# audioku/meta-transfer-learning

Hardware: AMD Instinct MI355X
Metric: meta-steps/sec (higher is better)
Workload: dtype f32 (emulated: 3x3 conv + input Linear on 2 x fp16 pieces "h2" = 22 significand bits, big GEMMs and attention (d_k = 64) on 3 x bf16 pieces "x3" = exact fp32 operands, small products on fp32 MFMA, element-wise on VALU; fp32 accumulation everywhere)

## Files before the change

meta-transfer-learning_amd/csrc/mtl_mfma.hip:

```cpp
#include <cstdlib>
#include <type_traits>

#include "mtl_common.h"
#include "mtl_h2.h"
#include "mtl_conv_narrow.h"
#include "../../include/mtl_hip.h"

namespace {

constexpr int BK = 32;
constexpr int NT = 256;

template <int ROWS>
struct LdsK {
    static constexpr int LD = BK + 1;
    static constexpr int SIZE = ROWS * LD;
    static __device__ __forceinline__ int at(int row, int k) { return row * LD + k; }
};
template <int ROWS>
struct LdsMN {
    static constexpr int LD = ROWS + 4;
    static constexpr int SIZE = BK * LD;
    static __device__ __forceinline__ int at(int row, int k) { return k * LD + row; }
};
// ... 782 lines not shown
    mx = wave_max(mx);
    if ((threadIdx.x & 63) == 0) sh[threadIdx.x >> 6] = mx;
    __syncthreads();
    if (threadIdx.x == 0) hdr_f[1 + blockIdx.x] = fmaxf(fmaxf(sh[0], sh[1]), fmaxf(sh[2], sh[3]));
}

struct ConvX3P {
    const float* x;
    const uint8_t* am_in;
    const unsigned char* w3;
    const float* bias;
    const float* act;
    float* y;
    uint8_t* am_out;
    ConvGeom g;
    int ntile;
    int dbg;
    int ntf, ntt, tiles;
    const float* amax_in;
    float* amax_out;
    int Bt;
    long sW, sBias, sAmaxIn, sAmaxOut;
    const int* widths;
    int wshift;
#ifdef MTL_X3_PROF
    unsigned long long* prof;
#endif
};
#ifdef MTL_X3_PROF
static unsigned long long* g_x3_prof = nullptr;
extern "C" void mtl_x3_prof_set(void* buf) { g_x3_prof = (unsigned long long*)buf; }
#define X3_T(v) const unsigned long long v = __builtin_amdgcn_s_memtime()
#define X3_ACC(slot, a, b) prof_acc[slot] += (b) - (a)
#define X3_PROF_DECL unsigned long long prof_acc[8] = {0, 0, 0, 0, 0, 0, 0, 0}
#define X3_PROF_FLUSH()                                                                                    \
    if (p.prof && (threadIdx.x & 63) == 0) {                                                               \
        for (int k_ = 0; k_ < 8; ++k_) p.prof[((long)blockIdx.x * 16 + (threadIdx.x >> 6)) * 8 + k_] = prof_acc[k_]; \
    }
#else
#define X3_T(v)
#define X3_ACC(slot, a, b)
#define X3_PROF_DECL
#define X3_PROF_FLUSH()
#endif

constexpr int XH_HF = 18;

struct X3Tile {
    int b, n0, t0, f0;
};

inline int device_cu_count() {
    int dev = 0, n = 0;
    if (hipGetDevice(&dev) != hipSuccess || hipDeviceGetAttribute(&n, hipDeviceAttributeMultiprocessorCount, dev) != hipSuccess || n <= 0)
        n = 256;
    return n;
}

template <int G>
__device__ inline int x3_task_rows(const ConvX3P& p, int task) {
    const int r = ((p.widths[task] >> p.wshift) + 8 * G - 1) / (8 * G);
    return r < p.ntt ? (r < 1 ? 1 : r) : p.ntt;
}

template <int G>
__device__ inline int x3_total_tiles(const ConvX3P& p) {
    if (!p.widths) return p.tiles;
    const int nt = p.g.B / p.Bt;
    int total = 0;
    for (int k = 0; k < nt; ++k) total += p.Bt * p.ntile * x3_task_rows<G>(p, k) * p.ntf;
    return total;
}

struct X3Cur {
    int k = 0, lo = 0, hi = -1, ntt = 0;
};

template <int G>
__device__ inline X3Tile x3_tile(const ConvX3P& p, int id, X3Cur& c) {
    X3Tile t;
    int ntt = p.ntt, b0 = 0;
    if (p.widths) {
        const int per_row = p.Bt * p.ntile * p.ntf, nt = p.g.B / p.Bt;
        if (c.hi < 0 || id < c.lo) {
            c.k = 0;
            c.lo = 0;
            c.ntt = x3_task_rows<G>(p, 0);
            c.hi = per_row * c.ntt;
        }
        while (id >= c.hi && c.k < nt - 1) {
            ++c.k;
            c.lo = c.hi;
            c.ntt = x3_task_rows<G>(p, c.k);
            c.hi = c.lo + per_row * c.ntt;
        }
        id -= c.lo;
        ntt = c.ntt;
        b0 = c.k * p.Bt;
    }
    const int fx = id % p.ntf;
    id /= p.ntf;
    const int ty = id % ntt;
    id /= ntt;
    t.f0 = fx * 16;
    t.t0 = ty * (8 * G);
    t.n0 = id % p.ntile;
    t.b = b0 + id / p.ntile;
    return t;
}

template <bool SWZ>
__device__ __forceinline__ float x3_wave_max(float v) {
    if constexpr (!SWZ) {
        return wave_max(v);
    } else {
        v = fmaxf(v, __int_as_float(__builtin_amdgcn_ds_swizzle(__float_as_int(v), (1 << 10) | 0x1f)));
        v = fmaxf(v, __int_as_float(__builtin_amdgcn_ds_swizzle(__float_as_int(v), (2 << 10) | 0x1f)));
        v = fmaxf(v, __int_as_float(__builtin_amdgcn_ds_swizzle(__float_as_int(v), (4 << 10) | 0x1f)));
        v = fmaxf(v, __int_as_float(__builtin_amdgcn_ds_swizzle(__float_as_int(v), (8 << 10) | 0x1f)));
        v = fmaxf(v, __int_as_float(__builtin_amdgcn_ds_swizzle(__float_as_int(v), (16 << 10) | 0x1f)));
        return fmaxf(__int_as_float(__builtin_amdgcn_readlane(__float_as_int(v), 0)), __int_as_float(__builtin_amdgcn_readlane(__float_as_int(v), 32)));
    }
}
template <bool SWZ>
__device__ __forceinline__ float x3_amax_read(const float* a) {
    return x3_wave_max<SWZ>(a[(threadIdx.x & (MTL_AMAX_SLOTS - 1)) * MTL_AMAX_STRIDE]);
}
template <bool SWZ>
__device__ __forceinline__ void x3_amax_raise(float* a, float mx) {
    mx = x3_wave_max<SWZ>(mx);
    float* slot = a + (blockIdx.x & (MTL_AMAX_SLOTS - 1)) * MTL_AMAX_STRIDE;
    if ((threadIdx.x & 63) == 0 && mx > *slot) atomicMax(reinterpret_cast<unsigned*>(slot), __float_as_uint(mx));
}

template <int BN, int G, bool UNPOOL, int EPI, int NP, int WN>
constexpr bool x3h_slim_fwd() {
    return X3H_M16 != 0 && NP == 2 && G == 2 && !UNPOOL &&
           ((BN == 64 && WN == 1 && EPI != EPI_DGRAD) || (BN == 128 && WN == 2 && EPI == EPI_RELU));
}
template <int BN, int G, bool UNPOOL, int EPI, int NP, int WN>
constexpr bool x3h_slim_dg128() {
    return NP == 2 && G == 2 && UNPOOL && EPI == EPI_DGRAD && BN == 128 && WN == 2;
}
constexpr bool x3h_lane_offsets_fit(long ch) { return (15 * ch + 64) * 4 < (1L << 32); }
static_assert(x3h_lane_offsets_fit(128) && x3h_lane_offsets_fit(71582783) && !x3h_lane_offsets_fit(71582784), "just below / at the limit");
static_assert((15 * 71582783L + 63) * 4 + 7 <= 0xffffffffL, "the last byte a lane offset reaches below the limit");

template <int BN, int G, bool UNPOOL, int EPI, int NP, int WN, bool WIDE = false>
__global__ __launch_bounds__((2 * WN * G + 4) * 64) __attribute__((amdgpu_waves_per_eu(WN == 1 ? 4 : 1)))
void conv3x3_x3h_kernel(ConvX3P p) {
    constexpr bool SLIM_FWD = !WIDE && x3h_slim_fwd<BN, G, UNPOOL, EPI, NP, WN>();
    constexpr bool SLIM_H32 = WN == 1 && EPI == EPI_DGRAD;
    constexpr bool SLIM_DG = SLIM_H32 || (!WIDE && x3h_slim_dg128<BN, G, UNPOOL, EPI, NP, WN>());
    constexpr bool SLIM_HALO = SLIM_DG;
    constexpr bool SLIM = SLIM_DG || SLIM_FWD;
    constexpr int CW = 2 * WN;
    constexpr int WTM = 64, WTN = BN / WN, TM = WTM / 32, TN = WTN / 32;
    constexpr int XH_HT = 8 * G + 2, XH_NPIX = XH_HT * XH_HF;
    constexpr int XH_APLANE = XH_NPIX * X3_ROWB;
    constexpr int NHALO = 3 * 64;
    constexpr int XH_NVA = (XH_NPIX * 8 + NHALO - 1) / NHALO;
    constexpr int NCONS = CW * G * 64;
    constexpr int BPLANE = BN * 64, BBUF = NP * BPLANE, ABUF = NP * XH_APLANE;
    constexpr int NDMA = BBUF / 1024;
    extern __shared__ __attribute__((aligned(16))) unsigned char smx[];
    unsigned char* smA = smx;
    unsigned char* smB = smx + ABUF;
    const int tid = threadIdx.x;
    const int Cin = p.g.Cin, Cout = p.g.Cout, cch = Cin / BK, nk = 9 * cch;
    const int T = p.g.T, F = p.g.F, Tp = p.g.Tp, Fp = p.g.Fp;
    const int my_tiles = (x3_total_tiles<G>(p) - (int)blockIdx.x + (int)gridDim.x - 1) / (int)gridDim.x;
    if (my_tiles <= 0) return;
    const int nstage = my_tiles * cch;
    const int nstep = nstage * 9;

    if (tid >= NCONS + 64) {
        const int ptid = tid - NCONS - 64;
        float sx = NP == 2 ? pow2_scale(x3_amax_read<SLIM>(p.amax_in)) : 1.f;
        int sx_task = 0;
        X3Cur cur_scale, cur_halo;
        auto set_scale = [&](int qc) {
            if (NP != 2 || p.Bt >= p.g.B) return;
            const int tk = x3_tile<G>(p, blockIdx.x + (qc / cch) * gridDim.x, cur_scale).b / p.Bt;
            if (tk != sx_task) {
                sx_task = tk;
                sx = pow2_scale(x3_amax_read<SLIM>(p.amax_in + tk * p.sAmaxIn));
            }
        };
        float4 hv[XH_NVA];
        uchar4 ha[XH_NVA];
        unsigned hm[SLIM_HALO ? 1 : XH_NVA];
        auto fetch_halo = [&](int q) {
            const int j = q / cch, c = q - j * cch;
            const X3Tile tl = x3_tile<G>(p, blockIdx.x + j * gridDim.x, cur_halo);
            int pt = ptid;
            if constexpr (SLIM_HALO) asm volatile("" : "+v"(pt));
#pragma unroll
            for (int i = 0; i < XH_NVA; ++i) {
                const int e = pt + i * NHALO;
                const int hp = min(e >> 3, XH_NPIX - 1), c4 = (e & 7) * 4;
                const int ht = hp / XH_HF, hf = hp - ht * XH_HF;
                const int ts = tl.t0 + ht - 1, fs = tl.f0 + hf - 1;
                bool ok = (e >> 3) < XH_NPIX && (unsigned)ts < (unsigned)T && (unsigned)fs < (unsigned)F;
                const int tc = min(max(ts, 0), T - 1), fc = min(max(fs, 0), F - 1);
                if (!UNPOOL) {
                    hv[i] = *reinterpret_cast<const float4*>(p.x + (((long)tl.b * T + tc) * F + fc) * Cin + c * BK + c4);
                    if constexpr (SLIM_HALO) hm[0] = i ? hm[0] | ((ok ? 1u : 0u) << i) : (ok ? 1u : 0u);
                    else hm[i] = ok ? 1u : 0u;
                } else {
                    const int tp = tc >> 1, fp = fc >> 1;
                    ok = ok && tp < Tp && fp < Fp;
                    if constexpr (SLIM_H32) {
                        const long sbase = (long)__builtin_amdgcn_readfirstlane(tl.b) * Tp * Fp * Cin + c * BK;
                        const unsigned o = (unsigned)((min(tp, Tp - 1) * Fp + min(fp, Fp - 1)) * Cin + c4);
                        ha[i] = *reinterpret_cast<const uchar4*>(p.am_in + sbase + o);
                        hv[i] = *reinterpret_cast<const float4*>(reinterpret_cast<const char*>(p.x + sbase) + o * 4u);
                    } else {
                    const long o = (((long)tl.b * Tp + min(tp, Tp - 1)) * Fp + min(fp, Fp - 1)) * Cin + c * BK + c4;
                    ha[i] = *reinterpret_cast<const uchar4*>(p.am_in + o);
                    hv[i] = *reinterpret_cast<const float4*>(p.x + o);
                    }
                    if constexpr (SLIM_HALO) hm[0] = i ? hm[0] | ((ok ? 1u : 0u) << i) : (ok ? 1u : 0u);
                    else hm[i] = (ok ? 1u : 0u) | ((unsigned)(((fs & 1) << 1) | (ts & 1)) << 1);
                }
            }
        };
        auto commit_halo = [&]() {
            int pt = ptid;
            if constexpr (SLIM_HALO) asm volatile("" : "+v"(pt));
#pragma unroll
            for (int i = 0; i < XH_NVA; ++i) {
                const int e = pt + i * NHALO;
                if ((e >> 3) >= XH_NPIX) continue;
                float4 v = hv[i];
                const bool ok = SLIM_HALO ? (hm[0] >> i) & 1u : hm[i] & 1u;
                if (!UNPOOL) {
                    v = mask4(v, ok ? 15u : 0u);
                } else {
                    const int ht_ = (e >> 3) / XH_HF, hf_ = (e >> 3) - ht_ * XH_HF;
                    const unsigned sub = SLIM_HALO ? (unsigned)((((hf_ + 1) & 1) << 1) | ((ht_ + 1) & 1)) : hm[SLIM_HALO ? 0 : i] >> 1;
                    v.x = (ok && ha[i].x == sub) ? v.x : 0.f;
                    v.y = (ok && ha[i].y == sub) ? v.y : 0.f;
                    v.z = (ok && ha[i].z == sub) ? v.z : 0.f;
                    v.w = (ok && ha[i].w == sub) ? v.w : 0.f;
                }
                uint2 pc[NP];
                split_x4<NP>(v, sx, pc);
                unsigned char* dst = smA + (e >> 3) * X3_ROWB + (e & 7) * 8;
#pragma unroll
                for (int q = 0; q < NP; ++q) *reinterpret_cast<uint2*>(dst + q * XH_APLANE) = pc[q];
            }
        };
        const bool doA = !(p.dbg & 2);
        X3_PROF_DECL;
        X3_T(h0);
        if (doA) fetch_halo(0);
        set_scale(0);
        if (doA) commit_halo();
        if (nstage > 1 && doA) fetch_halo(1);
        __syncthreads();
        X3_T(h1);
        X3_ACC(0, h0, h1);
#pragma unroll 1
        for (int q = 0; q < nstage; ++q) {
            X3_T(a0);
#pragma unroll 1
            for (int tap = 0; tap < 9; ++tap) __syncthreads();
            X3_T(a1);
            X3_ACC(1, a0, a1);
            if (q + 1 < nstage) {
                set_scale(q + 1);
                if (doA) commit_halo();
                X3_T(a2);
                X3_ACC(2, a1, a2);
                if (q + 2 < nstage && doA) fetch_halo(q + 2);
                X3_T(a3);
                X3_ACC(3, a2, a3);
                __syncthreads();
                X3_T(a4);
                X3_ACC(4, a3, a4);
            }
        }
        X3_PROF_FLUSH();
        return;
    }
    if (tid >= NCONS) {
        const int lane = tid & 63;
        const bool doB = !(p.dbg & 4);
        int dma_j = -1, dma_n0 = 0;
        X3Cur cur_dma;
        const unsigned char* dma_w3 = p.w3;
        auto dma = [&](int s_) {
            const int q = s_ / 9, tap = s_ - q * 9;
            const int j = q / cch, c = q - j * cch;
            if (j != dma_j && (p.ntile != 1 || p.Bt < p.g.B)) {
                const X3Tile tl = x3_tile<G>(p, blockIdx.x + j * gridDim.x, cur_dma);
                dma_n0 = tl.n0 * BN;
                dma_w3 = p.w3 + (tl.b / p.Bt) * p.sW;
                dma_j = j;
            }
            const int n0 = dma_n0;
            const unsigned char* w3 = dma_w3;
            const int kt = tap * cch + c;
            unsigned char* dst = smB + (s_ % 3) * BBUF;
#pragma unroll
            for (int i = 0; i < NDMA; ++i) {
                const int piece = i / (BN / 16), r16 = i - piece * (BN / 16);
                const unsigned char* g = w3 + (((long)piece * nk + kt) * Cout + n0 + r16 * 16) * 64 + lane * 16;
                __builtin_amdgcn_global_load_lds((const __attribute__((address_space(1))) void*)g,
                                                 (__attribute__((address_space(3))) void*)(dst + i * 1024), 16, 0, 0);
            }
        };
        if (doB) {
            dma(0);
            if (nstep > 1) dma(1);
        }
        if (nstep > 1) asm volatile("s_waitcnt vmcnt(%0)" ::"n"(NDMA) : "memory");
        else asm volatile("s_waitcnt vmcnt(0)" ::: "memory");
        __builtin_amdgcn_s_barrier();
        int tap = 0, q = 0;
        X3_PROF_DECL;
#pragma unroll 1
        for (int s_ = 0; s_ < nstep; ++s_) {
            X3_T(w0);
            if (s_ + 2 < nstep) {
                if (doB) dma(s_ + 2);
                X3_T(w1);
                X3_ACC(0, w0, w1);
                asm volatile("s_waitcnt vmcnt(%0)" ::"n"(NDMA) : "memory");
                X3_T(w2);
                X3_ACC(1, w1, w2);
            } else {
                asm volatile("s_waitcnt vmcnt(0)" ::: "memory");
            }
            X3_T(w3);
            __builtin_amdgcn_s_barrier();
            X3_T(w4);
            X3_ACC(2, w3, w4);
            if (++tap == 9) {
                tap = 0;
                if (++q < nstage) __builtin_amdgcn_s_barrier();
                X3_T(w5);
                X3_ACC(3, w4, w5);
            }
        }
        X3_PROF_FLUSH();
        return;
    }

    const int lane = tid & 63, wave = tid >> 6;
    const int grp = wave / CW, w4 = wave % CW;
    const int wm = w4 / WN, wn = w4 % WN, l31 = lane & 31, hi = lane >> 5;
    constexpr bool M16 = X3H_M16 != 0 && !(BN == 64 && G == 2 && (WN == 2 || X3H_DG5 != 2) && EPI == EPI_DGRAD && !UNPOOL);
    constexpr int TM16 = WTM / 16, TN16 = WTN / 16;
    constexpr int DGB16 = 2, DGB32 = 1;
    f32x16 acc[M16 ? 1 : TM][M16 ? 1 : TN];
    f32x4 acc4[M16 ? TM16 : 1][M16 ? TN16 : 1];
    const int l15 = lane & 15, q4 = lane >> 4;
    float inv = 1.f, mx = 0.f;
    if (NP == 2) inv = 1.f / (pow2_scale(x3_amax_read<SLIM>(p.amax_in)) * *reinterpret_cast<const float*>(p.w3 + (long)NP * nk * Cout * 64));
    int cur_task = 0;
    X3Cur cur_epi;
    const float* bias_t = p.bias;
    auto raise_bound = [&]() {
        if (!p.amax_out) return;
        float bmax = 0.f;
        if constexpr (SLIM_FWD) {
            int c15;
            asm volatile("v_mbcnt_lo_u32_b32 %0, -1, 0\n\tv_mbcnt_hi_u32_b32 %0, -1, %0" : "=v"(c15));
            const float* bias_k = p.bias + (long)cur_task * p.sBias + wn * WTN + 2 * (c15 & 15);
#pragma unroll
            for (int jn = 0; jn < TN16; ++jn)
                for (int nt = 0; nt < p.ntile; ++nt) bmax = fmaxf(bmax, fabsf(bias_k[nt * BN + (jn >> 1) * 32 + (jn & 1)]));
        } else
        if (EPI != EPI_DGRAD) {
            if (M16) {
#pragma unroll
                for (int jn = 0; jn < TN16; ++jn)
                    for (int nt = 0; nt < p.ntile; ++nt)
                        bmax = fmaxf(bmax, fabsf(bias_t[nt * BN + wn * WTN + (jn >> 1) * 32 + 2 * l15 + (jn & 1)]));
            } else
#pragma unroll
            for (int jn = 0; jn < TN; ++jn)
                for (int nt = 0; nt < p.ntile; ++nt) bmax = fmaxf(bmax, fabsf(bias_t[nt * BN + wn * WTN + jn * 32 + l31]));
        }
        x3_amax_raise<SLIM>(p.amax_out + cur_task * p.sAmaxOut, mx + bmax);
    };
    int abase[TM];
#pragma unroll
    for (int i = 0; i < TM; ++i) {
        int t, f;
        tile_row_to_tf(wm * WTM + i * 32 + l31, t, f);
        abase[i] = ((t + grp * 8 + 1) * XH_HF + (f + 1)) * X3_ROWB + hi * 16;
#ifdef X3_FAKE_A
        abase[i] = (XH_HF + 1 + l31 + i * 32 + grp * 64) * X3_ROWB + hi * 16;
#endif
    }
    int abase16[M16 ? TM16 : 1];
// ... 1259 lines not shown
int mtl_conv3x3_relu_pool_fwd(void* stream, const float* x, const float* w_fwd, const float* bias, float* p_out,
                              unsigned char* argmax, int B, int T, int F, int Cin, int Cout) {
    if (!x || !w_fwd || !bias || !p_out || !argmax) return MTL_EINVAL;
    ConvP p{x, nullptr, w_fwd, bias, nullptr, p_out, argmax, {B, T, F, Cin, Cout, T / 2, F / 2}, 1};
    return dispatch_conv<false, EPI_POOL>(p, 2 * (T / 2), 2 * (F / 2), as_stream(stream));
}

int mtl_conv3x3_dgrad(void* stream, const float* dy, const unsigned char* argmax, const float* w_dgrad,
                      const float* act, float* dx, int B, int T, int F, int Cin, int Cout) {
    if (!dy || !w_dgrad || !act || !dx) return MTL_EINVAL;
    ConvP p{dy, argmax, w_dgrad, nullptr, act, dx, nullptr, {B, T, F, Cout, Cin, T / 2, F / 2}, 1};
    if (argmax) return dispatch_conv<true, EPI_DGRAD>(p, T, F, as_stream(stream));
    return dispatch_conv<false, EPI_DGRAD>(p, T, F, as_stream(stream));
}

}

static int wprep_pieces(int np, hipStream_t s, const float* w_ref, void* wf, void* wd, int Cout, int Cin) {
    if (!w_ref || !wf || !wd || Cin % 32 || Cout % 32) return MTL_EINVAL;
    const long total = 9L * Cin * Cout;
    unsigned short* f = reinterpret_cast<unsigned short*>(wf);
    unsigned short* d = reinterpret_cast<unsigned short*>(wd);
    if (np == 2) {
        hipLaunchKernelGGL(conv_wscale_kernel, dim3(WSCALE_PARTS), dim3(256), 0, s, w_ref, (int)total, reinterpret_cast<float*>(f + 2 * total));
        hipLaunchKernelGGL(conv_wprep_x3_kernel<2>, dim3(grid_for(total, 256)), dim3(256), 0, s, w_ref, f, d, Cout, Cin);
    } else {
        hipLaunchKernelGGL(conv_wprep_x3_kernel<3>, dim3(grid_for(total, 256)), dim3(256), 0, s, w_ref, f, d, Cout, Cin);
    }
    MTL_CHECK_LAUNCH();
    return MTL_OK;
}

struct WprepBatch {
    const float* w[3];
    unsigned short* wf[3];
    unsigned short* wd[3];
    int Cout[3], Cin[3];
    long sSrc, sDst[3];
};
__global__ __launch_bounds__(256) void conv_wscale_batch_kernel(WprepBatch b) {
    __shared__ float sh[4];
    const int L = blockIdx.y, total = 9 * b.Cin[L] * b.Cout[L];
    b.w[L] += blockIdx.z * b.sSrc;
    b.wf[L] = reinterpret_cast<unsigned short*>(reinterpret_cast<unsigned char*>(b.wf[L]) + blockIdx.z * b.sDst[L]);
    const float* w = b.w[L];
    float mx = 0.f;
    for (int e = (blockIdx.x * 256 + threadIdx.x) * 4; e < total; e += WSCALE_PARTS * 1024) {
        const float4 v = *reinterpret_cast<const float4*>(w + e);
        mx = fmaxf(fmaxf(mx, fmaxf(fabsf(v.x), fabsf(v.y))), fmaxf(fabsf(v.z), fabsf(v.w)));
    }
    mx = wave_max(mx);
    if ((threadIdx.x & 63) == 0) sh[threadIdx.x >> 6] = mx;
    __syncthreads();
    if (threadIdx.x == 0) reinterpret_cast<float*>(b.wf[L] + 2L * total)[1 + blockIdx.x] = fmaxf(fmaxf(sh[0], sh[1]), fmaxf(sh[2], sh[3]));
}
__global__ void conv_wprep_h2_batch_kernel(WprepBatch b) {
    const int L = blockIdx.y, Cin = b.Cin[L], Cout = b.Cout[L];
    const float* w = b.w[L] + blockIdx.z * b.sSrc;
    unsigned short* wf = reinterpret_cast<unsigned short*>(reinterpret_cast<unsigned char*>(b.wf[L]) + blockIdx.z * b.sDst[L]);
    unsigned short* wd = reinterpret_cast<unsigned short*>(reinterpret_cast<unsigned char*>(b.wd[L]) + blockIdx.z * b.sDst[L]);
    const int total = 9 * Cin * Cout;
    const int nkf = 9 * (Cin / 32), nkd = 9 * (Cout / 32);
    float* hf = reinterpret_cast<float*>(wf + 2L * total);
    float mx = 0.f;
#pragma unroll
    for (int i = 1; i <= WSCALE_PARTS; ++i) mx = fmaxf(mx, hf[i]);
    const float s = pow2_scale(mx);
    if (blockIdx.x == 0 && threadIdx.x == 0) {
        hf[0] = s;
        *reinterpret_cast<float*>(wd + 2L * total) = s;
    }
    for (int e = blockIdx.x * blockDim.x + threadIdx.x; e < total; e += gridDim.x * blockDim.x) {
        const int tap = e % 9;
        const int cin = (e / 9) % Cin;
        const int cout = e / (9 * Cin);
        unsigned pc[2];
        Split<2>::x2(w[e], 0.f, s, pc);
#pragma unroll
        for (int p = 0; p < 2; ++p) {
            const unsigned short v = (unsigned short)(pc[p] & 0xffffu);
            wf[(((long)p * nkf + tap * (Cin / 32) + (cin >> 5)) * Cout + cout) * 32 + x3_swz(cin & 31, cout)] = v;
            wd[(((long)p * nkd + (8 - tap) * (Cout / 32) + (cout >> 5)) * Cin + cin) * 32 + x3_swz(cout & 31, cin)] = v;
        }
    }
}

struct ConvTasks {
    int tasks;
    long sW, sBias, sAmaxIn, sAmaxOut;
    const int* widths = nullptr;
    int wshift = 0;
};
static inline void set_tasks(ConvX3P& p, int B, const ConvTasks& tk) {
    p.Bt = B;
    p.widths = tk.widths;
    p.wshift = tk.wshift;
    p.sW = tk.sW;
    p.sBias = tk.sBias;
    p.sAmaxIn = tk.sAmaxIn;
    p.sAmaxOut = tk.sAmaxOut;
}

template <int NP>
static int conv_fwd_pieces(hipStream_t s, const float* x, const float* amax_x, const void* w, const float* bias, float* y,
                           unsigned char* argmax, float* amax_y, bool pool, int B, int T, int F, int Cin, int Cout,
                           ConvTasks tk = ConvTasks{1, 0, 0, 0, 0}) {
    if (!x || !w || !bias || !y || (pool && !argmax) || (NP == 2 && !amax_x) || tk.tasks < 1 || B < 1) return MTL_EINVAL;
    ConvX3P p{x, nullptr, reinterpret_cast<const unsigned char*>(w), bias, nullptr, y, argmax, {B * tk.tasks, T, F, Cin, Cout, T / 2, F / 2}, 1};
    p.amax_in = amax_x;
    p.amax_out = amax_y;
    set_tasks(p, B, tk);
    if (pool) return dispatch_conv_x3<false, EPI_POOL, NP>(p, 2 * (T / 2), 2 * (F / 2), s);
    return dispatch_conv_x3<false, EPI_RELU, NP>(p, T, F, s);
}

constexpr int EDGE_PIX = 32;
constexpr int EDGE_C = 64;
constexpr int EDGE_SMEM = (3 * EDGE_C * EDGE_C + (EDGE_PIX + 2) * EDGE_C) * 4;
template <int NP>
__global__ __launch_bounds__(256) void conv_dgrad_edge_kernel(ConvX3P p) {
    constexpr int N = EDGE_C, K = EDGE_C;
    const int T = p.g.T, F = p.g.F, Tp = p.g.Tp, Fp = p.g.Fp;
    const int b = blockIdx.y, t0 = blockIdx.x * EDGE_PIX, tid = threadIdx.x;
    const int task = b / p.Bt;
    int rows = T;
    if (p.widths) rows = min(T, ((p.widths[task] >> p.wshift) + 7) / 8 * 8);
    if (t0 >= rows) return;
    extern __shared__ __attribute__((aligned(16))) float edge_lds[];
    float* Ws = edge_lds;
    float* src = edge_lds + 3 * K * N;
    const unsigned short* w = reinterpret_cast<const unsigned short*>(p.w3 + task * p.sW);
    constexpr int nk = 9 * (K / 32);
    const float inv_sw = NP == 2 ? 1.f / *reinterpret_cast<const float*>(p.w3 + task * p.sW + (long)NP * nk * N * 64) : 1.f;
#pragma unroll 1
    for (int e = tid; e < 3 * (K / 32) * N * 4; e += 256) {
        const int chunk = e & 3, n = (e >> 2) % N, kt = e / (4 * N);
        float v[8] = {};
#pragma unroll
        for (int q = 0; q < NP; ++q) {
            const uint4 raw = *reinterpret_cast<const uint4*>(w + ((long)q * nk + kt) * N * 32 + n * 32 + chunk * 8);
            const unsigned u[4] = {raw.x, raw.y, raw.z, raw.w};
#pragma unroll
            for (int j = 0; j < 8; ++j) {
                const unsigned short bits = (unsigned short)(u[j >> 1] >> (16 * (j & 1)));
                v[j] += NP == 2 ? (float)__builtin_bit_cast(_Float16, bits) : __builtin_bit_cast(float, (unsigned)bits << 16);
            }
        }
        const int kk0 = ((chunk ^ ((n >> 2) & 3)) << 3);
        const int kw = kt / (K / 32), kc = kt - kw * (K / 32);
#pragma unroll
        for (int j = 0; j < 8; ++j) Ws[(kw * K + kc * 32 + kk0 + j) * N + n] = v[j] * inv_sw;
    }
    const int fs = F - 2, fp = fs >> 1;
    for (int e = tid; e < (EDGE_PIX + 2) * K; e += 256) {
        const int r = e / K, k = e - r * K, ts = t0 + r - 1, tp = ts >> 1;
        float v = 0.f;
        if (ts >= 0 && ts < T && tp < Tp && fp < Fp) {
            const long o = (((long)b * Tp + tp) * Fp + fp) * K + k;
            const unsigned sub = (unsigned)(((fs & 1) << 1) | (ts & 1));
            v = p.am_in[o] == sub ? p.x[o] : 0.f;
        }
        src[e] = v;
    }
    __syncthreads();
    constexpr int PPG = EDGE_PIX / 4;
    const int n = tid & 63, grp = tid >> 6;
    float acc[PPG] = {};
#pragma unroll 1
    for (int kw = 0; kw < 3; ++kw)
#pragma unroll 2
        for (int k = 0; k < K; k += 4) {
            const float w0 = Ws[(kw * K + k) * N + n], w1 = Ws[(kw * K + k + 1) * N + n], w2 = Ws[(kw * K + k + 2) * N + n],
                        w3 = Ws[(kw * K + k + 3) * N + n];
#pragma unroll
            for (int i = 0; i < PPG; ++i) {
                const float4 sv = *reinterpret_cast<const float4*>(src + (grp * PPG + i + kw) * K + k);
                acc[i] += sv.x * w0 + sv.y * w1 + sv.z * w2 + sv.w * w3;
            }
        }
    float mx = 0.f;
#pragma unroll
    for (int i = 0; i < PPG; ++i) {
        const int t = t0 + grp * PPG + i;
        if (t < rows) {
            const long o = (((long)b * T + t) * F + (F - 1)) * N + n;
            const float v = p.act[o] > 0.f ? acc[i] : 0.f;
            p.y[o] = v;
            mx = fmaxf(mx, fabsf(v));
        }
    }
    if (p.amax_out) amax_raise(p.amax_out + task * p.sAmaxOut, mx);
}

template <int NP>
static int conv_dgrad_pieces(hipStream_t s, const float* dy, const float* amax_dy, const unsigned char* argmax, const void* w,
                             const float* act, float* dx, float* amax_dx, int B, int T, int F, int Cin, int Cout,
                             ConvTasks tk = ConvTasks{1, 0, 0, 0, 0}) {
    if (!dy || !w || !act || !dx || (NP == 2 && !amax_dy) || tk.tasks < 1 || B < 1) return MTL_EINVAL;
    ConvX3P p{dy, argmax, reinterpret_cast<const unsigned char*>(w), nullptr, act, dx, nullptr, {B * tk.tasks, T, F, Cout, Cin, T / 2, F / 2}, 1};
    p.amax_in = amax_dy;
    p.amax_out = amax_dx;
    set_tasks(p, B, tk);
    if (!argmax) return dispatch_conv_x3<false, EPI_DGRAD, NP>(p, T, F, s);
#ifndef MTL_DGRAD_EDGE
#define MTL_DGRAD_EDGE 1
#endif
    const bool edge = MTL_DGRAD_EDGE && (F & 1) && F >= 3 && T >= 1 && Cin == EDGE_C && Cout == EDGE_C && B * tk.tasks <= 65535;
    const int rc = dispatch_conv_x3<true, EPI_DGRAD, NP>(p, T, edge ? F - 1 : F, s);
    if (rc != MTL_OK || !edge) return rc;
    static int attr = set_smem(conv_dgrad_edge_kernel<NP>, EDGE_SMEM);
    if (attr) return attr;
    hipLaunchKernelGGL(conv_dgrad_edge_kernel<NP>, dim3((T + EDGE_PIX - 1) / EDGE_PIX, B * tk.tasks), dim3(256), EDGE_SMEM, s, p);
    MTL_CHECK_LAUNCH();
    return MTL_OK;
}

extern "C" {

int mtl_conv3x3_wprep_x3(void* stream, const float* w_ref, void* w3_fwd, void* w3_dgrad, int Cout, int Cin) {
    return wprep_pieces(3, as_stream(stream), w_ref, w3_fwd, w3_dgrad, Cout, Cin);
}

int mtl_conv3x3_relu_fwd_x3(void* stream, const float* x, const void* w3_fwd, const float* bias, float* y, int B, int T, int F,
                            int Cin, int Cout) {
    return conv_fwd_pieces<3>(as_stream(stream), x, nullptr, w3_fwd, bias, y, nullptr, nullptr, false, B, T, F, Cin, Cout);
}

int mtl_conv3x3_relu_pool_fwd_x3(void* stream, const float* x, const void* w3_fwd, const float* bias, float* p_out,
                                 unsigned char* argmax, int B, int T, int F, int Cin, int Cout) {
    return conv_fwd_pieces<3>(as_stream(stream), x, nullptr, w3_fwd, bias, p_out, argmax, nullptr, true, B, T, F, Cin, Cout);
}

int mtl_conv3x3_dgrad_x3(void* stream, const float* dy, const unsigned char* argmax, const void* w3_dgrad, const float* act,
                         float* dx, int B, int T, int F, int Cin, int Cout) {
    return conv_dgrad_pieces<3>(as_stream(stream), dy, nullptr, argmax, w3_dgrad, act, dx, nullptr, B, T, F, Cin, Cout);
}

static int wprep_h2_batch_sets(void* stream, int n, const float* w0, void* f0, void* d0, int Cout0, int Cin0, const float* w1, void* f1,
                               void* d1, int Cout1, int Cin1, const float* w2, void* f2, void* d2, int Cout2, int Cin2, int sets, long sSrc,
                               long sDst0, long sDst1, long sDst2) {
    if (n < 1 || n > 3 || sets < 1 || sets > 65535) return MTL_EINVAL;
    WprepBatch b{{w0, w1, w2},
                 {reinterpret_cast<unsigned short*>(f0), reinterpret_cast<unsigned short*>(f1), reinterpret_cast<unsigned short*>(f2)},
                 {reinterpret_cast<unsigned short*>(d0), reinterpret_cast<unsigned short*>(d1), reinterpret_cast<unsigned short*>(d2)},
                 {Cout0, Cout1, Cout2},
                 {Cin0, Cin1, Cin2},
                 sSrc,
                 {sDst0, sDst1, sDst2}};
    long tmax = 0;
    for (int i = 0; i < n; ++i) {
        if (!b.w[i] || !b.wf[i] || !b.wd[i] || b.Cin[i] % 32 || b.Cout[i] % 32 || b.Cin[i] <= 0 || b.Cout[i] <= 0) return MTL_EINVAL;
        if (sets > 1 && ((b.sDst[i] & 3) || (sSrc & 3))) return MTL_EINVAL;
        const long t = 9L * b.Cin[i] * b.Cout[i];
        tmax = t > tmax ? t : tmax;
    }
    hipStream_t s = as_stream(stream);
    hipLaunchKernelGGL(conv_wscale_batch_kernel, dim3(WSCALE_PARTS, n, sets), dim3(256), 0, s, b);
    hipLaunchKernelGGL(conv_wprep_h2_batch_kernel, dim3(grid_for(tmax, 256, 256), n, sets), dim3(256), 0, s, b);
    MTL_CHECK_LAUNCH();
    return MTL_OK;
}

int mtl_conv3x3_wprep_h2_batch(void* stream, int n, const float* w0, void* f0, void* d0, int Cout0, int Cin0, const float* w1, void* f1,
                               void* d1, int Cout1, int Cin1, const float* w2, void* f2, void* d2, int Cout2, int Cin2) {
    return wprep_h2_batch_sets(stream, n, w0, f0, d0, Cout0, Cin0, w1, f1, d1, Cout1, Cin1, w2, f2, d2, Cout2, Cin2, 1, 0, 0, 0, 0);
}

int mtl_conv3x3_wprep_h2_batch_tb(void* stream, int n, const float* w0, void* f0, void* d0, int Cout0, int Cin0, const float* w1, void* f1,
                                  void* d1, int Cout1, int Cin1, const float* w2, void* f2, void* d2, int Cout2, int Cin2, int sets,
                                  long sSrc, long sDst0, long sDst1, long sDst2) {
    return wprep_h2_batch_sets(stream, n, w0, f0, d0, Cout0, Cin0, w1, f1, d1, Cout1, Cin1, w2, f2, d2, Cout2, Cin2, sets, sSrc, sDst0, sDst1,
                               sDst2);
}

long mtl_conv3x3_wprep_h2_bytes(int Cout, int Cin) { return 2L * 9 * Cin * Cout * 2 + 4 * (1 + WSCALE_PARTS) + 12; }

int mtl_conv3x3_wprep_h2(void* stream, const float* w_ref, void* w2_fwd, void* w2_dgrad, int Cout, int Cin) {
    return wprep_pieces(2, as_stream(stream), w_ref, w2_fwd, w2_dgrad, Cout, Cin);
}

int mtl_conv3x3_relu_fwd_h2(void* stream, const float* x, const float* amax_x, const void* w2_fwd, const float* bias, float* y,
                            float* amax_y, int B, int T, int F, int Cin, int Cout) {
    return conv_fwd_pieces<2>(as_stream(stream), x, amax_x, w2_fwd, bias, y, nullptr, amax_y, false, B, T, F, Cin, Cout);
}

int mtl_conv3x3_relu_pool_fwd_h2(void* stream, const float* x, const float* amax_x, const void* w2_fwd, const float* bias,
                                 float* p_out, unsigned char* argmax, float* amax_p, int B, int T, int F, int Cin, int Cout) {
    return conv_fwd_pieces<2>(as_stream(stream), x, amax_x, w2_fwd, bias, p_out, argmax, amax_p, true, B, T, F, Cin, Cout);
}

int mtl_conv3x3_dgrad_h2(void* stream, const float* dy, const float* amax_dy, const unsigned char* argmax, const void* w2_dgrad,
                         const float* act, float* dx, float* amax_dx, int B, int T, int F, int Cin, int Cout) {
    return conv_dgrad_pieces<2>(as_stream(stream), dy, amax_dy, argmax, w2_dgrad, act, dx, amax_dx, B, T, F, Cin, Cout);
}

int mtl_conv3x3_relu_fwd_h2_tb(void* stream, const float* x, const float* amax_x, const void* w2_fwd, const float* bias, float* y,
                               float* amax_y, int B, int T, int F, int Cin, int Cout, int tasks, long sW, long sBias, long sAmaxX, long sAmaxY,
                               const int* widths, int wshift) {
    if (wshift < 0 || wshift > 8) return MTL_EINVAL;
    return conv_fwd_pieces<2>(as_stream(stream), x, amax_x, w2_fwd, bias, y, nullptr, amax_y, false, B, T, F, Cin, Cout,
                              ConvTasks{tasks, sW, sBias, sAmaxX, sAmaxY, widths, wshift});
}

int mtl_conv3x3_relu_pool_fwd_h2_tb(void* stream, const float* x, const float* amax_x, const void* w2_fwd, const float* bias, float* p_out,
                                    unsigned char* argmax, float* amax_p, int B, int T, int F, int Cin, int Cout, int tasks, long sW,
                                    long sBias, long sAmaxX, long sAmaxP, const int* widths, int wshift) {
    if (wshift < 0 || wshift > 8) return MTL_EINVAL;
    return conv_fwd_pieces<2>(as_stream(stream), x, amax_x, w2_fwd, bias, p_out, argmax, amax_p, true, B, T, F, Cin, Cout,
                              ConvTasks{tasks, sW, sBias, sAmaxX, sAmaxP, widths, wshift});
}

int mtl_conv3x3_dgrad_h2_tb(void* stream, const float* dy, const float* amax_dy, const unsigned char* argmax, const void* w2_dgrad,
                            const float* act, float* dx, float* amax_dx, int B, int T, int F, int Cin, int Cout, int tasks, long sW,
                            long sAmaxDy, long sAmaxDx, const int* widths, int wshift) {
    if (wshift < 0 || wshift > 8) return MTL_EINVAL;
// ... 205 lines not shown
```

Before: 20.32.

## Load pooled sources once per window when unpooling halo tiles

In the unpool (max-unpool backward/dgrad) path of the 3x3 conv kernel, the halo producer now fetches each pooled source element once per 2x2 window, instead of once per unpooled pixel. It then scatters the value into the up to four LDS positions using the argmax code as a mask on the split pieces. The edge-column kernel gets the same treatment, reading each pooled row once and writing two unpooled rows. This cuts redundant global loads and address math by about 4x (2x for the edge kernel), at the cost of more LDS stores per element and extra boundary logic.

```diff
diff --git a/meta-transfer-learning_amd/csrc/mtl_mfma.hip b/meta-transfer-learning_amd/csrc/mtl_mfma.hip
--- a/meta-transfer-learning_amd/csrc/mtl_mfma.hip
+++ b/meta-transfer-learning_amd/csrc/mtl_mfma.hip
@@ -958,7 +958,7 @@
     constexpr bool SLIM_FWD = !WIDE && x3h_slim_fwd<BN, G, UNPOOL, EPI, NP, WN>();
     constexpr bool SLIM_H32 = WN == 1 && EPI == EPI_DGRAD;
     constexpr bool SLIM_DG = SLIM_H32 || (!WIDE && x3h_slim_dg128<BN, G, UNPOOL, EPI, NP, WN>());
-    constexpr bool SLIM_HALO = SLIM_DG;
+    constexpr bool SLIM_HALO = SLIM_DG && !UNPOOL;
     constexpr bool SLIM = SLIM_DG || SLIM_FWD;
     constexpr int CW = 2 * WN;
     constexpr int WTM = 64, WTN = BN / WN, TM = WTM / 32, TN = WTN / 32;
@@ -993,63 +993,87 @@
                 sx = pow2_scale(x3_amax_read<SLIM>(p.amax_in + tk * p.sAmaxIn));
             }
         };
-        float4 hv[XH_NVA];
-        uchar4 ha[XH_NVA];
-        unsigned hm[SLIM_HALO ? 1 : XH_NVA];
+        constexpr int XW_WF = XH_HF / 2 + 1, XW_NW = (XH_HT / 2 + 1) * XW_WF;
+        constexpr int XW_NVA = (XW_NW * 8 + NHALO - 1) / NHALO;
+        constexpr int NVA = UNPOOL ? XW_NVA : XH_NVA;
+        float4 hv[NVA];
+        uchar4 ha[NVA];
+        unsigned hm[SLIM_HALO || UNPOOL ? 1 : XH_NVA];
         auto fetch_halo = [&](int q) {
             const int j = q / cch, c = q - j * cch;
             const X3Tile tl = x3_tile<G>(p, blockIdx.x + j * gridDim.x, cur_halo);
             int pt = ptid;
             if constexpr (SLIM_HALO) asm volatile("" : "+v"(pt));
+            if constexpr (UNPOOL) {
+                const int tw0 = (tl.t0 >> 1) - 1, fw0 = (tl.f0 >> 1) - 1;
+#pragma unroll
+                for (int i = 0; i < XW_NVA; ++i) {
+                    const int e = pt + i * NHALO;
+                    const int w = min(e >> 3, XW_NW - 1), c4 = (e & 7) * 4;
+                    const int wr = w / XW_WF, wc = w - wr * XW_WF;
+                    const int tp = tw0 + wr, fp = fw0 + wc;
+                    const bool ok = (e >> 3) < XW_NW && (unsigned)tp < (unsigned)Tp && (unsigned)fp < (unsigned)Fp;
+                    const int tpc = max(min(tp, Tp - 1), 0), fpc = max(min(fp, Fp - 1), 0);
+                    if constexpr (SLIM_H32) {
+                        const long sbase = (long)__builtin_amdgcn_readfirstlane(tl.b) * Tp * Fp * Cin + c * BK;
+                        const unsigned o = (unsigned)((tpc * Fp + fpc) * Cin + c4);
+                        ha[i] = *reinterpret_cast<const uchar4*>(p.am_in + sbase + o);
+                        hv[i] = *reinterpret_cast<const float4*>(reinterpret_cast<const char*>(p.x + sbase) + o * 4u);
+                    } else {
+                        const long o = (((long)tl.b * Tp + tpc) * Fp + fpc) * Cin + c * BK + c4;
+                        ha[i] = *reinterpret_cast<const uchar4*>(p.am_in + o);
+                        hv[i] = *reinterpret_cast<const float4*>(p.x + o);
+                    }
+                    hm[0] = i ? hm[0] | ((ok ? 1u : 0u) << i) : (ok ? 1u : 0u);
+                }
+                return;
+            }
 #pragma unroll
             for (int i = 0; i < XH_NVA; ++i) {
                 const int e = pt + i * NHALO;
                 const int hp = min(e >> 3, XH_NPIX - 1), c4 = (e & 7) * 4;
                 const int ht = hp / XH_HF, hf = hp - ht * XH_HF;
                 const int ts = tl.t0 + ht - 1, fs = tl.f0 + hf - 1;
-                bool ok = (e >> 3) < XH_NPIX && (unsigned)ts < (unsigned)T && (unsigned)fs < (unsigned)F;
+                const bool ok = (e >> 3) < XH_NPIX && (unsigned)ts < (unsigned)T && (unsigned)fs < (unsigned)F;
                 const int tc = min(max(ts, 0), T - 1), fc = min(max(fs, 0), F - 1);
-                if (!UNPOOL) {
-                    hv[i] = *reinterpret_cast<const float4*>(p.x + (((long)tl.b * T + tc) * F + fc) * Cin + c * BK + c4);
-                    if constexpr (SLIM_HALO) hm[0] = i ? hm[0] | ((ok ? 1u : 0u) << i) : (ok ? 1u : 0u);
-                    else hm[i] = ok ? 1u : 0u;
-                } else {
-                    const int tp = tc >> 1, fp = fc >> 1;
-                    ok = ok && tp < Tp && fp < Fp;
-                    if constexpr (SLIM_H32) {
-                        const long sbase = (long)__builtin_amdgcn_readfirstlane(tl.b) * Tp * Fp * Cin + c * BK;
-                        const unsigned o = (unsigned)((min(tp, Tp - 1) * Fp + min(fp, Fp - 1)) * Cin + c4);
-                        ha[i] = *reinterpret_cast<const uchar4*>(p.am_in + sbase + o);
-                        hv[i] = *reinterpret_cast<const float4*>(reinterpret_cast<const char*>(p.x + sbase) + o * 4u);
-                    } else {
-                    const long o = (((long)tl.b * Tp + min(tp, Tp - 1)) * Fp + min(fp, Fp - 1)) * Cin + c * BK + c4;
-                    ha[i] = *reinterpret_cast<const uchar4*>(p.am_in + o);
-                    hv[i] = *reinterpret_cast<const float4*>(p.x + o);
-                    }
-                    if constexpr (SLIM_HALO) hm[0] = i ? hm[0] | ((ok ? 1u : 0u) << i) : (ok ? 1u : 0u);
-                    else hm[i] = (ok ? 1u : 0u) | ((unsigned)(((fs & 1) << 1) | (ts & 1)) << 1);
-                }
+                hv[i] = *reinterpret_cast<const float4*>(p.x + (((long)tl.b * T + tc) * F + fc) * Cin + c * BK + c4);
+                if constexpr (SLIM_HALO) hm[0] = i ? hm[0] | ((ok ? 1u : 0u) << i) : (ok ? 1u : 0u);
+                else hm[i] = ok ? 1u : 0u;
             }
         };
         auto commit_halo = [&]() {
             int pt = ptid;
             if constexpr (SLIM_HALO) asm volatile("" : "+v"(pt));
+            if constexpr (UNPOOL) {
+#pragma unroll
+                for (int i = 0; i < XW_NVA; ++i) {
+                    const int e = pt + i * NHALO;
+                    if ((e >> 3) >= XW_NW) continue;
+                    const int wr = (e >> 3) / XW_WF, wc = (e >> 3) - wr * XW_WF;
+                    uint2 pc[NP];
+                    split_x4<NP>(hv[i], sx, pc);
+                    const uchar4 a = (hm[0] >> i) & 1u ? ha[i] : make_uchar4(255, 255, 255, 255);
+                    unsigned char* dst = smA + ((2 * wr - 1) * XH_HF + 2 * wc - 1) * X3_ROWB + (e & 7) * 8;
+#pragma unroll
+                    for (int pos = 0; pos < 4; ++pos) {
+                        const int dr = pos & 1, dc = pos >> 1;
+                        if ((dr ? wr < XH_HT / 2 : wr > 0) && (dc ? wc < XW_WF - 1 : wc > 0)) {
+                            const unsigned m0 = (a.x == pos ? 0xffffu : 0u) | (a.y == pos ? 0xffff0000u : 0u);
+                            const unsigned m1 = (a.z == pos ? 0xffffu : 0u) | (a.w == pos ? 0xffff0000u : 0u);
+#pragma unroll
+                            for (int q = 0; q < NP; ++q)
+                                *reinterpret_cast<uint2*>(dst + (dr * XH_HF + dc) * X3_ROWB + q * XH_APLANE) = make_uint2(pc[q].x & m0, pc[q].y & m1);
+                        }
+                    }
+                }
+                return;
+            }
 #pragma unroll
             for (int i = 0; i < XH_NVA; ++i) {
                 const int e = pt + i * NHALO;
                 if ((e >> 3) >= XH_NPIX) continue;
-                float4 v = hv[i];
                 const bool ok = SLIM_HALO ? (hm[0] >> i) & 1u : hm[i] & 1u;
-                if (!UNPOOL) {
-                    v = mask4(v, ok ? 15u : 0u);
-                } else {
-                    const int ht_ = (e >> 3) / XH_HF, hf_ = (e >> 3) - ht_ * XH_HF;
-                    const unsigned sub = SLIM_HALO ? (unsigned)((((hf_ + 1) & 1) << 1) | ((ht_ + 1) & 1)) : hm[SLIM_HALO ? 0 : i] >> 1;
-                    v.x = (ok && ha[i].x == sub) ? v.x : 0.f;
-                    v.y = (ok && ha[i].y == sub) ? v.y : 0.f;
-                    v.z = (ok && ha[i].z == sub) ? v.z : 0.f;
-                    v.w = (ok && ha[i].w == sub) ? v.w : 0.f;
-                }
+                const float4 v = mask4(hv[i], ok ? 15u : 0u);
                 uint2 pc[NP];
                 split_x4<NP>(v, sx, pc);
                 unsigned char* dst = smA + (e >> 3) * X3_ROWB + (e & 7) * 8;
@@ -2615,15 +2639,19 @@
         for (int j = 0; j < 8; ++j) Ws[(kw * K + kc * 32 + kk0 + j) * N + n] = v[j] * inv_sw;
     }
     const int fs = F - 2, fp = fs >> 1;
-    for (int e = tid; e < (EDGE_PIX + 2) * K; e += 256) {
-        const int r = e / K, k = e - r * K, ts = t0 + r - 1, tp = ts >> 1;
+    static_assert(EDGE_PIX % 2 == 0, "even row origins");
+    for (int e = tid; e < (EDGE_PIX / 2 + 2) * K; e += 256) {
+        const int wr = e / K, k = e - wr * K, tp = (t0 >> 1) - 1 + wr;
         float v = 0.f;
-        if (ts >= 0 && ts < T && tp < Tp && fp < Fp) {
+        unsigned code = 255u;
+        if (tp >= 0 && tp < Tp && fp < Fp) {
             const long o = (((long)b * Tp + tp) * Fp + fp) * K + k;
-            const unsigned sub = (unsigned)(((fs & 1) << 1) | (ts & 1));
-            v = p.am_in[o] == sub ? p.x[o] : 0.f;
-        }
-        src[e] = v;
+            v = p.x[o];
+            code = p.am_in[o];
+        }
+        const unsigned sub = (unsigned)((fs & 1) << 1);
+        if (wr > 0) src[(2 * wr - 1) * K + k] = code == sub ? v : 0.f;
+        if (wr <= EDGE_PIX / 2) src[2 * wr * K + k] = code == (sub | 1u) ? v : 0.f;
     }
     __syncthreads();
     constexpr int PPG = EDGE_PIX / 4;
```

Measured after the change: 20.58 (median of 6 runs). 1.01x the previous value.
